# nvlong21/Lightweight-face-detection-CenterNet

Measured on AMD Instinct MI355X. Metric: images/sec at 640x640 batch inference, higher is better.
Workload: dtype bf16; 1 GPU; BASELINE configs[1]: batch=64 640x640 bf16 on 1 MI355X per rank, forward + top-100 peak decode; synthetic uint8 images resident in HBM, calibrated synthetic weights (seed 0); 2 context(s) per GPU, batch k on context k mod 2; batch_per_gpu=64, global_batch=64, topk=100, parallelism=dp1, contexts_per_gpu=2, input_buffers=4

## Files before the change

lightweight-face-detection-centernet_amd/csrc/cf_uphead.hip:

```cpp
#include "cf_exp.h"
#include "cf_common.h"
#include "cf_kernels.h"
#include <cstdlib>

namespace cf {

typedef __attribute__((ext_vector_type(8))) __bf16 mfma_bf16x8;

constexpr int UH_TW = 32, UH_IW = UH_TW + 2;

template <typename T, int UH_TH, int NW>
struct Uh {
    static constexpr int P = Elem<T>::PER16;
    static constexpr int PIT = 24 * (int)sizeof(T);
    static constexpr int NC = PIT / 16, NCH = (NC + 1) / 2;
    static constexpr int CPD = 3 * NC, SPD = (CPD + 1) / 2;
    static constexpr int G = 16 / P;
    static constexpr int IH = UH_TH + 2, IPX = IH * UH_IW, NIB = (IPX + 31) / 32, MAXB = (NIB + NW - 1) / NW;
    static constexpr int T3B = NIB * 32 * PIT, WHB = 3 * SPD * 1024, RSB = NW * 2048;
    static constexpr int LDS = T3B + WHB + RSB;
};

template <typename T, bool COALESCE, int UH_TH = 8, int NW = 4, bool NT = false>
__global__ __launch_bounds__(NW * 64) void uphead_kernel(UpHeadParams p) {
    typedef Uh<T, UH_TH, NW> U;
    constexpr int P = U::P, PIT = U::PIT, NC = U::NC, NCH = U::NCH, CPD = U::CPD, SPD = U::SPD, G = U::G;
    constexpr int UH_IPX = U::IPX, UH_NIB = U::NIB, MAXB = U::MAXB;
    extern __shared__ __attribute__((aligned(16))) char smem[];
    char* T3 = smem;
    char* Wh = smem + U::T3B;
    char* Rs = Wh + U::WHB;
    const int tid = threadIdx.x, lane = tid & 63, wave = tid >> 6;
    const int pl = lane & 31, h = lane >> 5;
    unsigned tbx = blockIdx.x, tby = blockIdx.y, tbz = blockIdx.z;
    if (p.xcd) xcd_tile_order(tbx, tby, tbz);
    const int ox0 = tbx * UH_TW, oy0 = tby * UH_TH, b = tbz;

    for (int c = wave; c < U::WHB / 1024; c += NW)
        __builtin_amdgcn_global_load_lds((const __attribute__((address_space(1))) void*)((const char*)p.w0p + c * 1024 + lane * 16),
                                         (__attribute__((address_space(3))) void*)(Wh + c * 1024), 16, 0, 0);

    u32x4 wc[NCH];
#pragma unroll
    for (int j = 0; j < NCH; ++j) wc[j] = ld16((const char*)p.wcv + (size_t)(j * 64 + lane) * 16);
    u32x4 xs[MAXB][NCH], lw[MAXB][G];
    bool valid[MAXB]; int tapv[MAXB];
#pragma unroll
    for (int t = 0; t < MAXB; ++t) {
        const int ib = wave + NW * t;
        const int ip = ib * 32 + pl;
        const int ipc = ip < UH_IPX ? ip : UH_IPX - 1;
        const int ty = ipc / UH_IW, tx = ipc - ty * UH_IW;
        const int gy = oy0 - 1 + ty, gx = ox0 - 1 + tx;
        valid[t] = ib < UH_NIB && ip < UH_IPX && (unsigned)gy < (unsigned)p.h && (unsigned)gx < (unsigned)p.w;
        const int cy = min(max(gy, 0), p.h - 1), cx = min(max(gx, 0), p.w - 1);
        const char* xrow = (const char*)p.skip + (((size_t)b * p.h + cy) * p.w + cx) * PIT;
#pragma unroll
        for (int j = 0; j < NCH; ++j) xs[t][j] = ld16(xrow + min(h * NCH + j, NC - 1) * 16);
        const size_t low_row = ((size_t)b * (p.h >> 1) + (cy >> 1)) * (p.w >> 1) + (cx >> 1);
        tapv[t] = ((cy & 1) << 1) | (cx & 1);
#pragma unroll
        for (int g = 0; g < G; ++g) lw[t][g] = ld16((const char*)p.low + (low_row * 24 + min(h * 16 + g * P, 24 - P)) * sizeof(T));
    }
#pragma unroll
    for (int t = 0; t < MAXB; ++t) {
        const int ib = wave + NW * t;
        if (ib >= UH_NIB) break;
        const int ip = ib * 32 + pl;
        f32x16 acc;
#pragma unroll
        for (int r = 0; r < 16; ++r) acc[r] = 0.0f;
        mma_chain<T, NCH>(acc, [&](int j) { return wc[j]; }, [&](int j) { return (h * NCH + j) < NC ? xs[t][j] : zero16(); });
        const int tap = tapv[t];
#pragma unroll
        for (int g = 0; g < G; ++g) {
            const int ch = h * 16 + g * P;
            if (ch >= 24) break;
            float v[P], r[P];
#pragma unroll
            for (int e = 0; e < P; ++e) v[e] = relu_f(acc[g * P + e] + p.bias[ch + e]);
            unpack16<T>(lw[t][g], r);
#pragma unroll
            for (int e = 0; e < P; ++e) v[e] += relu_f(r[e] * p.upw[tap * 24 + ch + e] + p.upb[ch + e]);
            u32x4 o = pack16<T>(v);
            if (!valid[t]) o = zero16();
            st16(T3 + ip * PIT + ch * (int)sizeof(T), o);
        }
    }
    cf_sync_lds_dma();

    for (int ob = wave; ob < UH_TH * UH_TW / 32; ob += NW) {
        const int o = ob * 32 + pl;
        const int oy = o / UH_TW, ox = o - oy * UH_TW;
        f32x16 acc;
#pragma unroll
        for (int r = 0; r < 16; ++r) acc[r] = 0.0f;
#pragma unroll
        for (int dy = 0; dy < 3; ++dy) {
            const char* row = T3 + ((oy + dy) * UH_IW + ox) * PIT;
            mma_chain<T, SPD>(acc, [&](int j) { return ld16(Wh + ((dy * SPD + j) * 64 + lane) * 16); },
                              [&](int j) { const int c = h * SPD + j; u32x4 xc = ld16(row + (c < CPD ? c : CPD - 1) * 16);
                                           if (c >= CPD) xc = zero16(); return xc; });
        }
        const int gy = oy0 + oy, gx = ox0 + ox;
        if constexpr (!COALESCE) { if (gy >= p.h || gx >= p.w) continue; }
        float out[8];
#pragma unroll
        for (int r = 0; r < 4; ++r) { out[r] = acc[r] + p.b0[h * 4 + r]; out[4 + r] = acc[4 + r] + p.b0[8 + h * 4 + r]; }
        const size_t m = ((size_t)b * p.h + gy) * p.w + gx;
        const bool inmap = gy < p.h && gx < p.w;
        if (h == 0) {
            float sg = 1.0f / (1.0f + expf(-out[0]));
            sg = fminf(fmaxf(sg, 1e-4f), 1.0f - 1e-4f);
            out[0] = sg;
            if (p.hm_plane && inmap) p.hm_plane[m] = sg;
        }
        if constexpr (COALESCE) {
            char* rs = Rs + wave * 2048;
            st16(rs + pl * 64 + h * 16, pack16<float>(&out[0]));
            st16(rs + pl * 64 + 32 + h * 16, pack16<float>(&out[4]));
            __builtin_amdgcn_wave_barrier();
            if (gy < p.h) {
                char* row0 = (char*)(p.heads + (((size_t)b * p.h + gy) * p.w + ox0) * 16);
#pragma unroll
                for (int k = 0; k < 2; ++k) {
                    const int q = lane + 64 * k;
                    const u32x4 v = ld16(rs + q * 16);
                    if (ox0 + (q >> 2) < p.w) {
                        if constexpr (NT) __builtin_nontemporal_store(v, reinterpret_cast<u32x4*>(row0 + q * 16));
                        else st16(row0 + q * 16, v);
                    }
                }
            }
            __builtin_amdgcn_wave_barrier();
        }
        if constexpr (!COALESCE) {
            float* dst = p.heads + m * 16 + h * 4;
            st16(dst, pack16<float>(&out[0]));
            st16(dst + 8, pack16<float>(&out[4]));
        }
    }
}

template <typename T, bool CO, int TH, int NW, bool NT>
static hipError_t uphead_launch_t(hipStream_t s, const UpHeadParams& q) {
    typedef Uh<T, TH, NW> U;
    dim3 grid((q.w + UH_TW - 1) / UH_TW, (q.h + TH - 1) / TH, q.B), blk(NW * 64);
    set_kernel_tag("void cf::uphead_kernel<%s, %s, %d, %d, %s>(cf::UpHeadParams)", type_tag<T>(), CO ? "true" : "false", TH, NW, NT ? "true" : "false");
    return launch_lds<uphead_kernel<T, CO, TH, NW, NT>>(grid, blk, U::LDS, s, q);
}

hipError_t launch_uphead(hipStream_t s, int dtype, const UpHeadParams& p) {
    if (p.B <= 0) return hipSuccess;
    static const bool xcd_on = cf_ab_int("CF_UH_XCD", 0) >= 1;
    UpHeadParams q = p; q.xcd = xcd_on ? 1 : 0;
#include CF_EXP_INC(cf_uphead_0)
    if (dtype == 1) return uphead_launch_t<bf16_t, true, 16, 8, true>(s, q);
    if (dtype == 2) return uphead_launch_t<sp32_t, true, 8, 8, true>(s, q);
    return uphead_launch_t<float, true, 8, 4, true>(s, q);
}

}
```

lightweight-face-detection-centernet_amd/csrc/experiments/cf_uphead_0.inc:

```
    static const int var = cf_ab_int("CF_UH_VARIANT", 0);
    if (dtype == 1) {
        if (cf_ab_int("CF_UH_COALESCE", 1) == 0) return uphead_launch_t<bf16_t, false, 8, 4, false>(s, q);
        switch (var) {
            case 1: return uphead_launch_t<bf16_t, true, 8, 4, true>(s, q);
            case 2: return uphead_launch_t<bf16_t, true, 16, 8, false>(s, q);
            case 3: return uphead_launch_t<bf16_t, true, 8, 4, false>(s, q);
            case 4: return uphead_launch_t<bf16_t, true, 16, 4, true>(s, q);
            case 5: return uphead_launch_t<bf16_t, true, 32, 8, true>(s, q);
            case 6: return uphead_launch_t<bf16_t, true, 8, 8, true>(s, q);
            default: break;
        }
    } else if (dtype == 2) {
        switch (var) {
            case 1: return uphead_launch_t<sp32_t, true, 8, 4, true>(s, q);
            case 2: return uphead_launch_t<sp32_t, true, 16, 8, true>(s, q);
            case 3: return uphead_launch_t<sp32_t, true, 4, 4, true>(s, q);
            case 4: return uphead_launch_t<sp32_t, true, 16, 16, true>(s, q);
            default: break;
        }
    }
```

Measured before the change: 54870 images/s.

## Add persistent run-based uphead kernel reusing halo rows and prefetching next tile

```diff
diff --git a/lightweight-face-detection-centernet_amd/csrc/cf_uphead.hip b/lightweight-face-detection-centernet_amd/csrc/cf_uphead.hip
--- a/lightweight-face-detection-centernet_amd/csrc/cf_uphead.hip
+++ b/lightweight-face-detection-centernet_amd/csrc/cf_uphead.hip
@@ -1,6 +1,8 @@
 #include "cf_exp.h"
 #include "cf_common.h"
 #include "cf_kernels.h"
+#include <algorithm>
+#include <atomic>
 #include <cstdlib>
 
 namespace cf {
@@ -142,6 +144,202 @@
     }
 }
 
+struct UhRuns {
+    typedef Uh<bf16_t, 16, 8> U;
+    static constexpr int NW = 8, TH = 16, IH = TH + 2;
+    static constexpr int TBF = 24 + 96 + 24 + 16;
+    static constexpr int TB_OFF = U::LDS, WC_OFF = TB_OFF + TBF * 4, LDS = WC_OFF + 2048;
+    static constexpr int ROW_B = UH_IW * U::PIT;
+    static constexpr int SHARED_CHUNKS = 2 * ROW_B / 16;
+    static_assert(U::MAXB == 3 && U::NIB == 20 && U::NCH == 2 && U::G == 2 && U::SPD == 5 && U::CPD == 9, "written out for this geometry");
+    static_assert(SHARED_CHUNKS <= NW * 64 && WC_OFF % 16 == 0 && TB_OFF % 16 == 0, "one chunk per thread; 16-byte LDS reads");
+};
+
+__device__ __forceinline__ void uh_lds_barrier() { asm volatile("s_waitcnt lgkmcnt(0)\n\ts_barrier" ::: "memory"); }
+
+typedef __amdgpu_buffer_rsrc_t uh_rsrc_t;
+constexpr unsigned UH_OOB = 0x80000000u;
+__device__ __forceinline__ uh_rsrc_t uh_rsrc(const void* base, int bytes) {
+    return __builtin_amdgcn_make_buffer_rsrc(const_cast<void*>(base), 0, bytes, 0x00020000);
+}
+typedef __attribute__((ext_vector_type(4))) unsigned int uh_v4u;
+__device__ __forceinline__ u32x4 uh_bload(uh_rsrc_t r, unsigned off) {
+    return __builtin_bit_cast(u32x4, __builtin_amdgcn_raw_buffer_load_b128(r, (int)off, 0, 0));
+}
+__device__ __forceinline__ void uh_bstore_nt(const u32x4& v, uh_rsrc_t r, unsigned off) {
+    __builtin_amdgcn_raw_buffer_store_b128(__builtin_bit_cast(uh_v4u, v), r, (int)off, 0, 2);
+}
+__device__ __forceinline__ void uh_bstore32(unsigned v, uh_rsrc_t r, unsigned off) {
+    __builtin_amdgcn_raw_buffer_store_b32(v, r, (int)off, 0, 0);
+}
+
+__global__ __launch_bounds__(UhRuns::NW * 64) __attribute__((amdgpu_waves_per_eu(4)))
+void uphead_runs_kernel(UpHeadParams p, int TX, int TY, unsigned tq, unsigned tr) {
+    typedef UhRuns R;
+    typedef R::U U;
+    typedef bf16_t T;
+    constexpr int PIT = U::PIT, NW = R::NW, UH_TH = R::TH;
+    extern __shared__ __attribute__((aligned(16))) char smem[];
+    char* T3 = smem;
+    char* Wh = smem + U::T3B;
+    char* Rs = Wh + U::WHB;
+    float* Tb = reinterpret_cast<float*>(smem + R::TB_OFF);
+    char* Wc = smem + R::WC_OFF;
+    const int tid = threadIdx.x, lane = tid & 63, wave = __builtin_amdgcn_readfirstlane(tid >> 6);
+    const int pl = lane & 31, h = lane >> 5;
+
+    const unsigned G = gridDim.x, wg = blockIdx.x;
+    unsigned t = wg * tq + wg * tr / G;
+    const unsigned t1 = (wg + 1) * tq + (wg + 1) * tr / G;
+    int b, col, row;
+    { const unsigned per = (unsigned)(TX * TY), bi = t / per, rem = t - bi * per, ci = rem / (unsigned)TY;
+      b = (int)bi; col = (int)ci; row = (int)(rem - ci * (unsigned)TY); }
+
+    int tyx[3];
+    const int wl = p.w >> 1;
+#pragma unroll
+    for (int k = 0; k < 3; ++k) {
+        const int ip = (wave + NW * k) * 32 + pl;
+        const int ty = ip / UH_IW, tx = ip - ty * UH_IW;
+        tyx[k] = (ty << 8) | tx;
+    }
+    const int cell0 = (wave * 32 + pl) * PIT;
+    const char* brow = T3 + (wave * UH_IW + pl) * PIT + h * (U::SPD * 16);
+
+    u32x4 xs[3][2], lw[3][2];
+    auto bounds = [&](int col_, int row_, int& ylo, int& ynum, int& xlo, int& xnum) {
+        const int oy0 = row_ * UH_TH, ox0 = col_ * UH_TW;
+        ylo = oy0 == 0 ? 1 : 0; ynum = min(R::IH, p.h - oy0 + 1) - ylo;
+        xlo = ox0 == 0 ? 1 : 0; xnum = min(UH_IW, p.w - ox0 + 1) - xlo;
+    };
+    auto issue = [&](int b_, int col_, int row_, bool shared, bool any) {
+        int ylo, ynum, xlo, xnum; bounds(col_, row_, ylo, ynum, xlo, xnum);
+        const int oy0 = row_ * UH_TH, ox0 = col_ * UH_TW;
+        const long long sb = (((long long)b_ * p.h + oy0 - 1) * p.w + ox0 - 1) * PIT;
+        const long long lb = (((long long)b_ * (p.h >> 1) + (oy0 >> 1) - 1) * wl + (ox0 >> 1) - 1) * PIT;
+        const uh_rsrc_t sk = uh_rsrc((const char*)p.skip + sb, any ? (R::IH * p.w + UH_IW) * PIT : 0);
+        const uh_rsrc_t lo = uh_rsrc((const char*)p.low + lb, any ? ((R::IH / 2 + 1) * wl + UH_IW / 2 + 1) * PIT : 0);
+#pragma unroll
+        for (int k = 0; k < 3; ++k) {
+            const int ty = tyx[k] >> 8, tx = tyx[k] & 255;
+            const bool ok = (unsigned)(ty - ylo) < (unsigned)ynum && (unsigned)(tx - xlo) < (unsigned)xnum && !(shared && wave + NW * k < 2);
+            const unsigned xo = ok ? (unsigned)((ty * p.w + tx) * PIT + h * 32) : UH_OOB;
+            const unsigned lo_ = ok ? (unsigned)((((ty + 1) >> 1) * wl + ((tx + 1) >> 1)) * PIT + h * 32) : UH_OOB;
+            xs[k][0] = uh_bload(sk, xo); lw[k][0] = uh_bload(lo, lo_);
+            xs[k][1] = uh_bload(sk, h == 0 ? xo + 16 : UH_OOB); lw[k][1] = uh_bload(lo, h == 0 ? lo_ + 16 : UH_OOB);
+        }
+    };
+    auto phase_a = [&](int col_, int row_, bool shared) {
+        int ylo, ynum, xlo, xnum; bounds(col_, row_, ylo, ynum, xlo, xnum);
+#pragma unroll
+        for (int k = 0; k < 3; ++k) {
+            const int ib = wave + NW * k;
+            if (ib >= U::NIB) break;
+            if (shared && ib < 2) continue;
+            const int ty = tyx[k] >> 8, tx = tyx[k] & 255;
+            const bool valid = (unsigned)(ty - ylo) < (unsigned)ynum && (unsigned)(tx - xlo) < (unsigned)xnum;
+            const bool keep = !(shared && ty < 2);
+            f32x16 acc;
+#pragma unroll
+            for (int r = 0; r < 16; ++r) acc[r] = 0.0f;
+            mma_chain<T, 2>(acc, [&](int j) { return ld16(Wc + (j * 64 + lane) * 16); }, [&](int j) { return xs[k][j]; });
+            const int tap = (((ty + 1) & 1) << 1) | ((tx + 1) & 1);
+#pragma unroll
+            for (int g = 0; g < 2; ++g) {
+                const int ch = h * 16 + g * 8;
+                if (ch >= 24) break;
+                float v[8], r[8];
+                unpack16<T>(lw[k][g], r);
+#pragma unroll
+                for (int q = 0; q < 8; q += 4) {
+                    float bs[4], uw[4], ub[4];
+                    unpack16<float>(ld16(Tb + ch + q), bs);
+                    unpack16<float>(ld16(Tb + 24 + tap * 24 + ch + q), uw);
+                    unpack16<float>(ld16(Tb + 120 + ch + q), ub);
+#pragma unroll
+                    for (int e = 0; e < 4; ++e) v[q + e] = relu_f(acc[g * 8 + q + e] + bs[e]);
+#pragma unroll
+                    for (int e = 0; e < 4; ++e) v[q + e] += relu_f(r[q + e] * uw[e] + ub[e]);
+                    __builtin_amdgcn_sched_barrier(0);
+                }
+                u32x4 o = pack16<T>(v);
+                if (!valid) o = zero16();
+                if (keep) st16(T3 + cell0 + k * (NW * 32 * PIT) + ch * (int)sizeof(T), o);
+            }
+        }
+    };
+
+    issue(b, col, row, false, true);
+    for (int c = wave; c < U::WHB / 1024; c += NW)
+        __builtin_amdgcn_global_load_lds((const __attribute__((address_space(1))) void*)((const char*)p.w0p + c * 1024 + lane * 16),
+                                         (__attribute__((address_space(3))) void*)(Wh + c * 1024), 16, 0, 0);
+    if (wave < 2)
+        __builtin_amdgcn_global_load_lds((const __attribute__((address_space(1))) void*)((const char*)p.wcv + wave * 1024 + lane * 16),
+                                         (__attribute__((address_space(3))) void*)(Wc + wave * 1024), 16, 0, 0);
+    if (tid < R::TBF) Tb[tid] = tid < 24 ? p.bias[tid] : tid < 120 ? p.upw[tid - 24] : tid < 144 ? p.upb[tid - 120] : p.b0[tid - 144];
+
+    asm volatile("s_waitcnt vmcnt(0)" ::: "memory");
+    uh_lds_barrier();
+    phase_a(col, row, false);
+    for (;;) {
+        uh_lds_barrier();
+
+        const bool more = t + 1 < t1;
+        int nb = b, ncol = col, nrow = row + 1;
+        bool nshared = more;
+        if (nrow == TY) { nrow = 0; nshared = false; if (++ncol == TX) { ncol = 0; ++nb; } }
+        issue(nb, ncol, nrow, nshared, more);
+
+        const int ox0 = col * UH_TW, oy0 = row * UH_TH;
+        const int wcells = min(UH_TW, p.w - ox0);
+#pragma unroll
+        for (int i = 0; i < 2; ++i) {
+            const int oy = wave + NW * i;
+            f32x16 acc;
+#pragma unroll
+            for (int r = 0; r < 16; ++r) acc[r] = 0.0f;
+#pragma unroll
+            for (int dy = 0; dy < 3; ++dy) {
+                const char* rp = brow + (NW * i + dy) * R::ROW_B;
+                mma_chain<T, 5>(acc, [&](int j) { return ld16(Wh + ((dy * 5 + j) * 64 + lane) * 16); },
+                                [&](int j) { u32x4 xc = ld16(rp + j * 16); if (j == 4 && h) xc = zero16(); return xc; });
+            }
+            const int gy = oy0 + oy;
+            float b0a[4], b0b[4], out[8];
+            unpack16<float>(ld16(Tb + 144 + h * 4), b0a); unpack16<float>(ld16(Tb + 152 + h * 4), b0b);
+#pragma unroll
+            for (int r = 0; r < 4; ++r) { out[r] = acc[r] + b0a[r]; out[4 + r] = acc[4 + r] + b0b[r]; }
+            if (h == 0) {
+                float sg = 1.0f / (1.0f + expf(-out[0]));
+                sg = fminf(fmaxf(sg, 1e-4f), 1.0f - 1e-4f);
+                out[0] = sg;
+            }
+            const size_t mrow = ((size_t)b * p.h + gy) * p.w + ox0;
+            const int ncell = gy < p.h ? wcells : 0;
+            uh_bstore32(__float_as_uint(out[0]), uh_rsrc(p.hm_plane + mrow, p.hm_plane ? ncell * 4 : 0), h == 0 ? (unsigned)(pl * 4) : UH_OOB);
+            char* rs = Rs + wave * 2048;
+            st16(rs + pl * 64 + h * 16, pack16<float>(&out[0]));
+            st16(rs + pl * 64 + 32 + h * 16, pack16<float>(&out[4]));
+            __builtin_amdgcn_wave_barrier();
+            const uh_rsrc_t hr = uh_rsrc(p.heads + mrow * 16, ncell * 64);
+#pragma unroll
+            for (int k = 0; k < 2; ++k) {
+                const int q = lane + 64 * k;
+                uh_bstore_nt(ld16(rs + q * 16), hr, (unsigned)(q * 16));
+            }
+            __builtin_amdgcn_wave_barrier();
+        }
+        if (!more) break;
+        u32x4 keep2 = zero16();
+        const bool copies = nshared && tid < R::SHARED_CHUNKS;
+        if (copies) keep2 = ld16(T3 + (R::IH - 2) * R::ROW_B + tid * 16);
+        uh_lds_barrier();
+        if (copies) st16(T3 + tid * 16, keep2);
+        b = nb; col = ncol; row = nrow; ++t;
+        phase_a(col, row, nshared);
+    }
+}
+
 template <typename T, bool CO, int TH, int NW, bool NT>
 static hipError_t uphead_launch_t(hipStream_t s, const UpHeadParams& q) {
     typedef Uh<T, TH, NW> U;
@@ -150,12 +348,33 @@
     return launch_lds<uphead_kernel<T, CO, TH, NW, NT>>(grid, blk, U::LDS, s, q);
 }
 
+static int uphead_slots() {
+    static std::atomic<int> cus[32];
+    int dev = 0; (void)hipGetDevice(&dev);
+    std::atomic<int>& slot = cus[dev & 31];
+    int n = slot.load(std::memory_order_relaxed);
+    if (n <= 0) {
+        if (hipDeviceGetAttribute(&n, hipDeviceAttributeMultiprocessorCount, dev) != hipSuccess || n <= 0) n = 1;
+        slot.store(n, std::memory_order_relaxed);
+    }
+    return 2 * std::min(n, 16384);
+}
+
+static hipError_t uphead_runs_launch(hipStream_t s, const UpHeadParams& q) {
+    const int TX = (q.w + UH_TW - 1) / UH_TW, TY = (q.h + UhRuns::TH - 1) / UhRuns::TH;
+    const long long T = (long long)TX * TY * q.B;
+    if (T > 0x7fffffffLL) return hipErrorInvalidValue;
+    const unsigned G = (unsigned)std::min<long long>(T, uphead_slots());
+    set_kernel_tag("cf::uphead_runs_kernel(cf::UpHeadParams, int, int, unsigned int, unsigned int)");
+    return launch_lds<uphead_runs_kernel>(dim3(G), dim3(UhRuns::NW * 64), UhRuns::LDS, s, q, TX, TY, (unsigned)(T / G), (unsigned)(T % G));
+}
+
 hipError_t launch_uphead(hipStream_t s, int dtype, const UpHeadParams& p) {
     if (p.B <= 0) return hipSuccess;
     static const bool xcd_on = cf_ab_int("CF_UH_XCD", 0) >= 1;
     UpHeadParams q = p; q.xcd = xcd_on ? 1 : 0;
 #include CF_EXP_INC(cf_uphead_0)
-    if (dtype == 1) return uphead_launch_t<bf16_t, true, 16, 8, true>(s, q);
+    if (dtype == 1) return uphead_runs_launch(s, q);
     if (dtype == 2) return uphead_launch_t<sp32_t, true, 8, 8, true>(s, q);
     return uphead_launch_t<float, true, 8, 4, true>(s, q);
 }
diff --git a/lightweight-face-detection-centernet_amd/csrc/experiments/cf_uphead_0.inc b/lightweight-face-detection-centernet_amd/csrc/experiments/cf_uphead_0.inc
--- a/lightweight-face-detection-centernet_amd/csrc/experiments/cf_uphead_0.inc
+++ b/lightweight-face-detection-centernet_amd/csrc/experiments/cf_uphead_0.inc
@@ -1,5 +1,6 @@
     static const int var = cf_ab_int("CF_UH_VARIANT", 0);
     if (dtype == 1) {
+        if (cf_ab_int("CF_UH_RUNS", 1) == 0) return uphead_launch_t<bf16_t, true, 16, 8, true>(s, q);
         if (cf_ab_int("CF_UH_COALESCE", 1) == 0) return uphead_launch_t<bf16_t, false, 8, 4, false>(s, q);
         switch (var) {
             case 1: return uphead_launch_t<bf16_t, true, 8, 4, true>(s, q);
```

Measured after the change: 55760 images/s (median of 6 runs). 1.6% higher.
